# zhangyk18/GeoBi-GNN

Hardware: AMD Instinct MI355X
Metric: M-edges/s (fwd+bwd) on Synthetic set (higher is better)
Workload: dtype f32; 1 GPU; Synthetic train, batch=4 meshes (~20k faces each), fwd+bwd [BASELINE.json configs[2]]: per rank 4 noisy icospheres n=32 (F=20480) as one disjoint-union graph, L1/L1 loss, grad all-reduce + Adam step inside the timed region; ONE resident batch replayed every step, its level-0 CSR / reverse-edge index / corner lists / loss weights built in warm-up and cached per mesh (with --full, extra.fresh_batch:; meshes_per_rank=4, edges_per_rank_step=1351448, parallelism=dp1, mesh_groups_in_flight=1, split_allreduce=False, collective=none

## Files before the change

### geobi_gnn_amd/csrc/head_fused.hip

```cpp
#include "common.h"

#include <cstdlib>

namespace geobi {

namespace {

typedef float f32x16 __attribute__((ext_vector_type(16)));

constexpr int CIN = 32;
constexpr int HID = 1024;
constexpr int NCHUNK = HID / 32;
constexpr float kEps = 1e-12f;

__device__ __forceinline__ int acc_row(int r, int half) { return (r & 3) + 8 * (r >> 2) + 4 * half; }

__device__ __forceinline__ void load16(const float* __restrict__ p, float (&v)[16]) {
  const float4* q = reinterpret_cast<const float4*>(p);
#pragma unroll
  for (int i = 0; i < 4; ++i) {
    float4 t = q[i];
    v[4 * i] = t.x; v[4 * i + 1] = t.y; v[4 * i + 2] = t.z; v[4 * i + 3] = t.w;
  }
}

template <int NOUT>
__global__ __launch_bounds__(256) void head_fwd_fused_kernel(
    const float* __restrict__ x, int N, const float* __restrict__ w1, const float* __restrict__ b1,
    const float* __restrict__ w2, const float* __restrict__ b2, float slope, int mode,
    const float* __restrict__ dd, const float* __restrict__ resid, int ld_resid, float* __restrict__ raw,
    float* __restrict__ out) {
  __shared__ float s_part[4][32][NOUT + 1];
  const int lane = threadIdx.x & 63, wave = threadIdx.x >> 6;
  const int half = lane >> 5, l31 = lane & 31;
  const int n0 = blockIdx.x * 32;
  const int row = min(n0 + l31, N - 1);
  float ax[16];
  load16(x + (size_t)row * CIN + 16 * half, ax);

  float part[16][NOUT];
#pragma unroll
  for (int r = 0; r < 16; ++r)
#pragma unroll
    for (int o = 0; o < NOUT; ++o) part[r][o] = 0.f;

  auto chunk = [&](int c, const float (&bw)[16]) {
    const int j = c * 32 + l31;
    f32x16 acc;
#pragma unroll
    for (int r = 0; r < 16; ++r) acc[r] = 0.f;
#pragma unroll
    for (int s = 0; s < 16; ++s) acc = __builtin_amdgcn_mfma_f32_32x32x2f32(ax[s], bw[s], acc, 0, 0, 0);
    const float b1v = b1[j];
    float w2v[NOUT];
#pragma unroll
    for (int o = 0; o < NOUT; ++o) w2v[o] = w2[(size_t)o * HID + j];
#pragma unroll
    for (int r = 0; r < 16; ++r) {
      float h = acc[r] + b1v;
      h = h > 0.f ? h : h * slope;
#pragma unroll
      for (int o = 0; o < NOUT; ++o) part[r][o] = fmaf(h, w2v[o], part[r][o]);
    }
  };
  const float* w1l = w1 + (size_t)l31 * CIN + 16 * half;
  float bwa[16], bwb[16];
  load16(w1l + (size_t)wave * 32 * CIN, bwa);
  for (int c = wave; c < NCHUNK; c += 8) {
    load16(w1l + (size_t)(c + 4) * 32 * CIN, bwb);
    chunk(c, bwa);
    if (c + 8 < NCHUNK) load16(w1l + (size_t)(c + 8) * 32 * CIN, bwa);
    chunk(c + 4, bwb);
  }
#pragma unroll
  for (int r = 0; r < 16; ++r)
#pragma unroll
    for (int o = 0; o < NOUT; ++o) {
      float v = part[r][o];
#pragma unroll
      for (int m = 16; m >= 1; m >>= 1) v += __shfl_xor(v, m, 64);
      part[r][o] = v;
    }
#pragma unroll
  for (int r = 0; r < 16; ++r) {
    if (l31 != r) continue;
#pragma unroll
    for (int o = 0; o < NOUT; ++o) s_part[wave][acc_row(r, half)][o] = part[r][o];
  }
  __syncthreads();
  if (threadIdx.x < 32) {
    const int node = n0 + threadIdx.x;
    if (node >= N) return;
    float v[NOUT];
#pragma unroll
    for (int o = 0; o < NOUT; ++o) {
      v[o] = ((s_part[0][threadIdx.x][o] + s_part[1][threadIdx.x][o]) + s_part[2][threadIdx.x][o]) +
             s_part[3][threadIdx.x][o] + b2[o];
      raw[(size_t)node * NOUT + o] = v[o];
    }
    float res[3];
    if (mode == 0) {
#pragma unroll
      for (int cidx = 0; cidx < 3; ++cidx) {
        float t = (NOUT == 3) ? v[cidx % NOUT] : v[0] * dd[(size_t)node * 3 + cidx];
        res[cidx] = t + resid[(size_t)node * ld_resid + cidx];
      }
    } else {
      float len = fmaxf(sqrtf(v[0] * v[0] + v[1 % NOUT] * v[1 % NOUT] + v[2 % NOUT] * v[2 % NOUT]), kEps);
#pragma unroll
      for (int cidx = 0; cidx < 3; ++cidx) res[cidx] = v[cidx % NOUT] / len;
    }
    out[(size_t)node * 3] = res[0]; out[(size_t)node * 3 + 1] = res[1]; out[(size_t)node * 3 + 2] = res[2];
  }
}

typedef __bf16 bf16x8 __attribute__((ext_vector_type(8)));

struct Split3 { bf16x8 p[3]; };

__device__ __forceinline__ Split3 split3(const float (&v)[8]) {
  Split3 o;
#pragma unroll
  for (int j = 0; j < 8; ++j) {
    const __bf16 a = (__bf16)v[j];
    const float r1 = v[j] - (float)a;
    const __bf16 b = (__bf16)r1;
    const float r2 = r1 - (float)b;
    o.p[0][j] = a; o.p[1][j] = b; o.p[2][j] = (__bf16)r2;
  }
  return o;
}

__device__ __forceinline__ void load8(const float* __restrict__ p, float (&v)[8]) {
  const float4* q = reinterpret_cast<const float4*>(p);
  const float4 a = q[0], b = q[1];
  v[0] = a.x; v[1] = a.y; v[2] = a.z; v[3] = a.w; v[4] = b.x; v[5] = b.y; v[6] = b.z; v[7] = b.w;
}

__device__ __forceinline__ f32x16 mfma6(const Split3& a, const Split3& b, f32x16 acc) {
  acc = __builtin_amdgcn_mfma_f32_32x32x16_bf16(a.p[2], b.p[0], acc, 0, 0, 0);
  acc = __builtin_amdgcn_mfma_f32_32x32x16_bf16(a.p[0], b.p[2], acc, 0, 0, 0);
  acc = __builtin_amdgcn_mfma_f32_32x32x16_bf16(a.p[1], b.p[1], acc, 0, 0, 0);
  acc = __builtin_amdgcn_mfma_f32_32x32x16_bf16(a.p[1], b.p[0], acc, 0, 0, 0);
  acc = __builtin_amdgcn_mfma_f32_32x32x16_bf16(a.p[0], b.p[1], acc, 0, 0, 0);
  acc = __builtin_amdgcn_mfma_f32_32x32x16_bf16(a.p[0], b.p[0], acc, 0, 0, 0);
  return acc;
}

__global__ void head_split_w1_kernel(const float* __restrict__ w1, __bf16* __restrict__ pk) {
  const int i = blockIdx.x * blockDim.x + threadIdx.x;
  if (i >= HID * CIN) return;
  const float v = w1[i];
  const __bf16 a = (__bf16)v;
  const float r1 = v - (float)a;
  const __bf16 b = (__bf16)r1;
  pk[i] = a; pk[HID * CIN + i] = b; pk[2 * HID * CIN + i] = (__bf16)(r1 - (float)b);
}

__device__ __forceinline__ Split3 load_split(const __bf16* __restrict__ pk, size_t off) {
  Split3 o;
#pragma unroll
  for (int p = 0; p < 3; ++p) o.p[p] = *reinterpret_cast<const bf16x8*>(pk + (size_t)p * HID * CIN + off);
  return o;
}

template <int NOUT>
__global__ __launch_bounds__(256) void head_fwd_fused_bf16x3_kernel(
    const float* __restrict__ x, int N, const __bf16* __restrict__ w1p, const float* __restrict__ b1,
    const float* __restrict__ w2, const float* __restrict__ b2, float slope, int mode,
    const float* __restrict__ dd, const float* __restrict__ resid, int ld_resid, float* __restrict__ raw,
    float* __restrict__ out) {
  __shared__ float s_part[4][32][NOUT + 1];
  const int lane = threadIdx.x & 63, wave = threadIdx.x >> 6;
  const int half = lane >> 5, l31 = lane & 31;
  const int n0 = blockIdx.x * 32;
  const int row = min(n0 + l31, N - 1);
  Split3 ax[2];
  {
    float v[8];
    load8(x + (size_t)row * CIN + 8 * half, v);      ax[0] = split3(v);
    load8(x + (size_t)row * CIN + 16 + 8 * half, v); ax[1] = split3(v);
  }
  float part[16][NOUT];
#pragma unroll
  for (int r = 0; r < 16; ++r)
#pragma unroll
    for (int o = 0; o < NOUT; ++o) part[r][o] = 0.f;

  auto chunk = [&](int c, const Split3& bw0, const Split3& bw1) {
    const int j = c * 32 + l31;
    f32x16 acc;
#pragma unroll
    for (int r = 0; r < 16; ++r) acc[r] = 0.f;
    acc = mfma6(ax[0], bw0, acc);
    acc = mfma6(ax[1], bw1, acc);
    const float b1v = b1[j];
    float w2v[NOUT];
#pragma unroll
    for (int o = 0; o < NOUT; ++o) w2v[o] = w2[(size_t)o * HID + j];
#pragma unroll
    for (int r = 0; r < 16; ++r) {
      float h = acc[r] + b1v;
      h = h > 0.f ? h : h * slope;
#pragma unroll
      for (int o = 0; o < NOUT; ++o) part[r][o] = fmaf(h, w2v[o], part[r][o]);
    }
  };
  const size_t wl = (size_t)l31 * CIN + 8 * half;
  Split3 wa0 = load_split(w1p, wl + (size_t)wave * 32 * CIN), wa1 = load_split(w1p, wl + (size_t)wave * 32 * CIN + 16);
  for (int c = wave; c < NCHUNK; c += 8) {
    const Split3 wb0 = load_split(w1p, wl + (size_t)(c + 4) * 32 * CIN), wb1 = load_split(w1p, wl + (size_t)(c + 4) * 32 * CIN + 16);
    chunk(c, wa0, wa1);
    if (c + 8 < NCHUNK) { wa0 = load_split(w1p, wl + (size_t)(c + 8) * 32 * CIN); wa1 = load_split(w1p, wl + (size_t)(c + 8) * 32 * CIN + 16); }
    chunk(c + 4, wb0, wb1);
  }
#pragma unroll
  for (int r = 0; r < 16; ++r)
#pragma unroll
    for (int o = 0; o < NOUT; ++o) {
      float v = part[r][o];
#pragma unroll
      for (int m = 16; m >= 1; m >>= 1) v += __shfl_xor(v, m, 64);
      part[r][o] = v;
    }
#pragma unroll
  for (int r = 0; r < 16; ++r) {
    if (l31 != r) continue;
#pragma unroll
    for (int o = 0; o < NOUT; ++o) s_part[wave][acc_row(r, half)][o] = part[r][o];
  }
  __syncthreads();
  if (threadIdx.x < 32) {
    const int node = n0 + threadIdx.x;
    if (node >= N) return;
    float v[NOUT];
#pragma unroll
    for (int o = 0; o < NOUT; ++o) {
      v[o] = ((s_part[0][threadIdx.x][o] + s_part[1][threadIdx.x][o]) + s_part[2][threadIdx.x][o]) +
             s_part[3][threadIdx.x][o] + b2[o];
      raw[(size_t)node * NOUT + o] = v[o];
    }
    float res[3];
    if (mode == 0) {
#pragma unroll
      for (int cidx = 0; cidx < 3; ++cidx) {
        float t = (NOUT == 3) ? v[cidx % NOUT] : v[0] * dd[(size_t)node * 3 + cidx];
        res[cidx] = t + resid[(size_t)node * ld_resid + cidx];
      }
    } else {
      float len = fmaxf(sqrtf(v[0] * v[0] + v[1 % NOUT] * v[1 % NOUT] + v[2 % NOUT] * v[2 % NOUT]), kEps);
#pragma unroll
      for (int cidx = 0; cidx < 3; ++cidx) res[cidx] = v[cidx % NOUT] / len;
    }
    out[(size_t)node * 3] = res[0]; out[(size_t)node * 3 + 1] = res[1]; out[(size_t)node * 3 + 2] = res[2];
  }
}

#ifdef GEOBI_HEAD_STAMPS
__device__ unsigned long long g_head_stamps[1024][8];
#define GEOBI_HS(i) do { const unsigned long long now_ = __builtin_amdgcn_s_memtime(); hs_acc[i] += now_ - hs_t; hs_t = now_; } while (0)
#else
#define GEOBI_HS(i) do { } while (0)
#endif

constexpr int HBW = 8;
constexpr int HCPW = NCHUNK / HBW;

template <int NOUT>
__global__ __launch_bounds__(512, 1) void head_bwd_fused_kernel(
    const float* __restrict__ x, int N, int ntiles, const float* __restrict__ w1, const float* __restrict__ b1,
    const float* __restrict__ w2, float slope, const float* __restrict__ graw, float* __restrict__ dx,
    float* __restrict__ p_dw1, float* __restrict__ p_dw2, float* __restrict__ p_db1, float* __restrict__ p_db2) {
  extern __shared__ __attribute__((aligned(16))) float lds[];
  float* sW1 = lds;
  float* sW2 = sW1 + NCHUNK * 16 * 64;
  float* sB1 = sW2 + 3 * HID;
  float* sT = sB1 + HID;
  const int lane = threadIdx.x & 63, wave = threadIdx.x >> 6;
  const int half = lane >> 5, l31 = lane & 31;
  for (int i = threadIdx.x; i < NCHUNK * 16 * 64 + 3 * HID + HID; i += 64 * HBW) lds[i] = 0.f;
  __syncthreads();

  float db2a[NOUT];
#pragma unroll
  for (int o = 0; o < NOUT; ++o) db2a[o] = 0.f;
  float* tw = sT + wave * 512;
#ifdef GEOBI_HEAD_STAMPS
  unsigned long long hs_acc[8] = {0, 0, 0, 0, 0, 0, 0, 0};
  unsigned long long hs_t = __builtin_amdgcn_s_memtime();
#endif

  for (int t = blockIdx.x; t < ntiles; t += gridDim.x) {
    const int n0 = t * 32;
    float ax[16], ax2[16], gr[16][NOUT];
    load16(x + (size_t)min(n0 + l31, N - 1) * CIN + 16 * half, ax);
#pragma unroll
    for (int r = 0; r < 16; ++r) {
      const int node = n0 + acc_row(r, half);
      const bool ok = node < N;
      ax2[r] = x[(size_t)(ok ? node : N - 1) * CIN + l31];
#pragma unroll
      for (int o = 0; o < NOUT; ++o) {
        gr[r][o] = ok ? graw[(size_t)node * NOUT + o] : 0.f;
        db2a[o] += gr[r][o];
      }
    }
    f32x16 dxacc;
#pragma unroll
    for (int r = 0; r < 16; ++r) dxacc[r] = 0.f;
    GEOBI_HS(0);

    float bw[16];
    load16(w1 + (size_t)(wave * 32 + l31) * CIN + 16 * half, bw);
    for (int cc = 0; cc < HCPW; ++cc) {
      const int c = wave + HBW * cc;
      const int j = c * 32 + l31;
      f32x16 acc;
#pragma unroll
      for (int r = 0; r < 16; ++r) acc[r] = 0.f;
#pragma unroll
      for (int s = 0; s < 16; ++s) acc = __builtin_amdgcn_mfma_f32_32x32x2f32(ax[s], bw[s], acc, 0, 0, 0);
      GEOBI_HS(1);
      float bq[16];
      const float* wq = w1 + (size_t)(c * 32 + 16 * half) * CIN + l31;
#pragma unroll
      for (int s = 0; s < 16; ++s) bq[s] = wq[s * CIN];
      const float b1v = b1[j];
      float w2v[NOUT], dw2c[NOUT];
#pragma unroll
      for (int o = 0; o < NOUT; ++o) { w2v[o] = w2[(size_t)o * HID + j]; dw2c[o] = 0.f; }
      load16(w1 + (size_t)((wave + HBW * ((cc + 1) % HCPW)) * 32 + l31) * CIN + 16 * half, bw);
      float dh[16];
      float db1c = 0.f;
#pragma unroll
      for (int r = 0; r < 16; ++r) {
        float hpre = acc[r] + b1v;
        float hval = hpre > 0.f ? hpre : hpre * slope;
        float gh = 0.f;
#pragma unroll
        for (int o = 0; o < NOUT; ++o) {
          gh = fmaf(gr[r][o], w2v[o], gh);
          dw2c[o] = fmaf(gr[r][o], hval, dw2c[o]);
        }
        dh[r] = hpre > 0.f ? gh : gh * slope;
        db1c += dh[r];
      }
      GEOBI_HS(2);
      f32x16 tacc;
#pragma unroll
      for (int r = 0; r < 16; ++r) tacc[r] = 0.f;
#pragma unroll
      for (int r = 0; r < 16; ++r) tacc = __builtin_amdgcn_mfma_f32_32x32x2f32(ax2[r], dh[r], tacc, 0, 0, 0);
      float ad[16];
#pragma unroll
      for (int pass = 0; pass < 2; ++pass) {
#pragma unroll
        for (int r8 = 0; r8 < 8; ++r8) {
          const int r = 8 * pass + r8;
          const int row = acc_row(r, half) - 16 * pass;
          tw[row * 32 + (l31 ^ ((row & 7) << 2))] = dh[r];
        }
        __builtin_amdgcn_fence(__ATOMIC_RELEASE, "wavefront");
        __builtin_amdgcn_wave_barrier();
        __builtin_amdgcn_fence(__ATOMIC_ACQUIRE, "wavefront");
        if ((l31 >> 4) == pass) {
          const int row = l31 & 15;
#pragma unroll
          for (int q = 0; q < 4; ++q) {
            float4 v = *reinterpret_cast<const float4*>(&tw[row * 32 + ((16 * half + 4 * q) ^ ((row & 7) << 2))]);
            ad[4 * q] = v.x; ad[4 * q + 1] = v.y; ad[4 * q + 2] = v.z; ad[4 * q + 3] = v.w;
          }
        }
        __builtin_amdgcn_fence(__ATOMIC_RELEASE, "wavefront");
        __builtin_amdgcn_wave_barrier();
        __builtin_amdgcn_fence(__ATOMIC_ACQUIRE, "wavefront");
      }
      GEOBI_HS(3);
#pragma unroll
      for (int s = 0; s < 16; ++s) dxacc = __builtin_amdgcn_mfma_f32_32x32x2f32(ad[s], bq[s], dxacc, 0, 0, 0);
      GEOBI_HS(4);
      db1c += __shfl_xor(db1c, 32, 64);
      if (half == 0) sB1[j] += db1c;
#pragma unroll
      for (int o = 0; o < NOUT; ++o) {
        float d = dw2c[o] + __shfl_xor(dw2c[o], 32, 64);
        if (half == 0) sW2[o * HID + j] += d;
      }
      float* w1c = sW1 + (size_t)c * 16 * 64 + lane;
#pragma unroll
      for (int r = 0; r < 16; ++r) w1c[r * 64] += tacc[r];
      GEOBI_HS(5);
    }
#pragma unroll
    for (int hr = 0; hr < 2; ++hr) {
      __syncthreads();
#pragma unroll
      for (int r8 = 0; r8 < 8; ++r8) sT[(wave * 8 + r8) * 64 + lane] = dxacc[8 * hr + r8];
      __syncthreads();
      {
        const int r8 = wave;
        float v = 0.f;
#pragma unroll
        for (int w = 0; w < HBW; ++w) v += sT[(w * 8 + r8) * 64 + lane];
        const int node = n0 + acc_row(8 * hr + r8, half);
        if (node < N) dx[(size_t)node * CIN + l31] = v;
      }
    }
    __syncthreads();
    GEOBI_HS(6);
  }
#ifdef GEOBI_HEAD_STAMPS
  if (threadIdx.x == 0 && blockIdx.x < 1024)
    for (int i = 0; i < 8; ++i) g_head_stamps[blockIdx.x][i] = hs_acc[i];
#endif

  __syncthreads();
  float* pw = p_dw1 + (size_t)blockIdx.x * (NCHUNK * 16 * 64);
  for (int i = threadIdx.x; i < NCHUNK * 16 * 64; i += 64 * HBW) pw[i] = sW1[i];
  for (int i = threadIdx.x; i < NOUT * HID; i += 64 * HBW) p_dw2[(size_t)blockIdx.x * NOUT * HID + i] = sW2[i];
  for (int i = threadIdx.x; i < HID; i += 64 * HBW) p_db1[(size_t)blockIdx.x * HID + i] = sB1[i];
  if (wave == 0) {
#pragma unroll
    for (int o = 0; o < NOUT; ++o) {
      float d = db2a[o] + __shfl_xor(db2a[o], 32, 64);
      if (lane == 0) p_db2[(size_t)blockIdx.x * 4 + o] = d;
    }
  }
}

__global__ __launch_bounds__(256) void head_bwd_reduce_kernel(const float* __restrict__ p_dw1, const float* __restrict__ p_dw2,
                                       const float* __restrict__ p_db1, const float* __restrict__ p_db2,
                                       int blocks, int nout, int accumulate, float* __restrict__ dw1,
                                       float* __restrict__ db1, float* __restrict__ dw2, float* __restrict__ db2) {
  __shared__ float part[4][64];
  const int o = threadIdx.x & 63, q = threadIdx.x >> 6;
  const int idx = blockIdx.x * 64 + o;
  const int n_dw1 = HID * CIN;
  const int total = n_dw1 + HID + nout * HID + nout;
  const float* src = nullptr;
  size_t stride = 0, off = 0;
  float* dst = nullptr;
  if (idx < n_dw1) {
    const int c = idx >> 10, r = (idx >> 6) & 15, lane = idx & 63;
    const int j = c * 32 + (lane & 31), k = acc_row(r, lane >> 5);
    src = p_dw1; stride = (size_t)NCHUNK * 16 * 64; off = idx; dst = dw1 + (size_t)j * CIN + k;
  } else if (idx < n_dw1 + HID) {
    src = p_db1; stride = HID; off = idx - n_dw1; dst = db1 + off;
  } else if (idx < n_dw1 + HID + nout * HID) {
    src = p_dw2; stride = (size_t)nout * HID; off = idx - n_dw1 - HID; dst = dw2 + off;
  } else if (idx < total) {
    src = p_db2; stride = 4; off = idx - n_dw1 - HID - nout * HID; dst = db2 + off;
  }
  float s = 0.f;
  if (src != nullptr) {
#pragma unroll 16
    for (int b = q; b < blocks; b += 4) s += src[(size_t)b * stride + off];
  }
  part[q][o] = s;
  __syncthreads();
  if (q == 0 && dst != nullptr) {
    const float t = ((part[0][o] + part[1][o]) + part[2][o]) + part[3][o];
    *dst = accumulate ? *dst + t : t;
  }
}

int bwd_blocks(int64_t N) {
  int ntiles = cdiv(N, 32);
  return ntiles < 256 ? ntiles : 256;
}

}

#ifdef GEOBI_HEAD_STAMPS
extern "C" int geobi_debug_head_stamps(void* host_dst, size_t bytes) {
  return (int)hipMemcpyFromSymbol(host_dst, HIP_SYMBOL(g_head_stamps), bytes, 0, hipMemcpyDeviceToHost);
}
#endif

bool head_fused_supported(int Cin, int K, int nout) { return Cin == CIN && K == HID && (nout == 1 || nout == 3); }

static std::atomic<int> g_head_precision{[] { const char* e = getenv("GEOBI_HEAD_BF16X3"); return (e && atoi(e) != 0) ? 1 : 0; }()};
int set_head_precision(int mode) {
  GEOBI_REQUIRE(mode == 0 || mode == 1, "head precision: 0 (fp32) or 1 (3 x bf16 split, six products)");
  g_head_precision = mode;
  return 0;
}

int head_fwd_fused(const float* x, int64_t N, const float* w1, const float* b1, const float* w2, const float* b2,
                   int nout, float slope, int mode, const float* dd, const float* resid, int ld_resid, float* raw,
                   float* out, hipStream_t s) {
  int blocks = cdiv(N, 32);
  if (g_head_precision.load(std::memory_order_relaxed) == 1) {
    static thread_local __bf16* pack = nullptr;
    if (pack == nullptr) GEOBI_HIP(hipMalloc((void**)&pack, (size_t)3 * HID * CIN * sizeof(__bf16)));
    head_split_w1_kernel<<<cdiv(HID * CIN, 256), 256, 0, s>>>(w1, pack);
    if (nout == 3)
      head_fwd_fused_bf16x3_kernel<3><<<blocks, 256, 0, s>>>(x, (int)N, pack, b1, w2, b2, slope, mode, dd, resid, ld_resid,
                                                             raw, out);
    else
      head_fwd_fused_bf16x3_kernel<1><<<blocks, 256, 0, s>>>(x, (int)N, pack, b1, w2, b2, slope, mode, dd, resid, ld_resid,
                                                             raw, out);
    GEOBI_LAUNCH_OK();
    return 0;
  }
  if (nout == 3)
    head_fwd_fused_kernel<3><<<blocks, 256, 0, s>>>(x, (int)N, w1, b1, w2, b2, slope, mode, dd, resid, ld_resid, raw,
                                                    out);
  else
    head_fwd_fused_kernel<1><<<blocks, 256, 0, s>>>(x, (int)N, w1, b1, w2, b2, slope, mode, dd, resid, ld_resid, raw,
                                                    out);
  GEOBI_LAUNCH_OK();
  return 0;
}

size_t head_bwd_fused_ws_bytes(int64_t N) {
  size_t b = bwd_blocks(N);
  return align_up(b * (size_t)NCHUNK * 16 * 64 * sizeof(float)) + align_up(b * 3 * HID * sizeof(float)) +
         align_up(b * HID * sizeof(float)) + align_up(b * 4 * sizeof(float)) + 1024;
}

int head_bwd_fused(const float* x, int64_t N, const float* w1, const float* b1, const float* w2, int nout,
                   float slope, const float* graw, float* dx, float* dw1, float* db1, float* dw2, float* db2,
                   int accumulate, void* ws, size_t ws_bytes, hipStream_t s) {
  const int blocks = bwd_blocks(N);
  Arena a(ws, ws_bytes);
  float* p_dw1 = a.take<float>((size_t)blocks * NCHUNK * 16 * 64);
  float* p_dw2 = a.take<float>((size_t)blocks * 3 * HID);
  float* p_db1 = a.take<float>((size_t)blocks * HID);
  float* p_db2 = a.take<float>((size_t)blocks * 4);
  GEOBI_REQUIRE(a.ok() && ws, "head_bwd_fused: workspace too small (%zu < %zu)", ws_bytes, a.off);
  const int ntiles = cdiv(N, 32);
  constexpr size_t kLds = (size_t)(NCHUNK * 16 * 64 + 3 * HID + HID + HBW * 16 * 32) * sizeof(float);
  static_assert(kLds == 163840, "the backward head kernel uses the whole LDS of a CU");
  static std::atomic<bool> attr_set{false};
  if (!attr_set) {
    GEOBI_HIP(hipFuncSetAttribute((const void*)head_bwd_fused_kernel<3>, hipFuncAttributeMaxDynamicSharedMemorySize,
                                  (int)kLds));
    GEOBI_HIP(hipFuncSetAttribute((const void*)head_bwd_fused_kernel<1>, hipFuncAttributeMaxDynamicSharedMemorySize,
                                  (int)kLds));
    attr_set = true;
  }
  if (nout == 3)
    head_bwd_fused_kernel<3><<<blocks, 64 * HBW, kLds, s>>>(x, (int)N, ntiles, w1, b1, w2, slope, graw, dx, p_dw1, p_dw2,
                                                       p_db1, p_db2);
  else
    head_bwd_fused_kernel<1><<<blocks, 64 * HBW, kLds, s>>>(x, (int)N, ntiles, w1, b1, w2, slope, graw, dx, p_dw1, p_dw2,
                                                       p_db1, p_db2);
  GEOBI_LAUNCH_OK();
  const int total = HID * CIN + HID + nout * HID + nout;
  head_bwd_reduce_kernel<<<cdiv(total, 64), 256, 0, s>>>(p_dw1, p_dw2, p_db1, p_db2, blocks, nout, accumulate, dw1, db1,
                                                          dw2, db2);
  GEOBI_LAUNCH_OK();
  return 0;
}

}
```

Before: 328.8 M-edges/s.

## Add tiled head forward and multi-subtile backward kernels with register-resident dW2/dB1

New measurement: 333.3 M-edges/s, median of 4. +1.4%, better.

```diff
diff --git a/geobi_gnn_amd/csrc/head_fused.hip b/geobi_gnn_amd/csrc/head_fused.hip
--- a/geobi_gnn_amd/csrc/head_fused.hip
+++ b/geobi_gnn_amd/csrc/head_fused.hip
@@ -96,6 +96,141 @@
     for (int o = 0; o < NOUT; ++o) {
       v[o] = ((s_part[0][threadIdx.x][o] + s_part[1][threadIdx.x][o]) + s_part[2][threadIdx.x][o]) +
              s_part[3][threadIdx.x][o] + b2[o];
+      raw[(size_t)node * NOUT + o] = v[o];
+    }
+    float res[3];
+    if (mode == 0) {
+#pragma unroll
+      for (int cidx = 0; cidx < 3; ++cidx) {
+        float t = (NOUT == 3) ? v[cidx % NOUT] : v[0] * dd[(size_t)node * 3 + cidx];
+        res[cidx] = t + resid[(size_t)node * ld_resid + cidx];
+      }
+    } else {
+      float len = fmaxf(sqrtf(v[0] * v[0] + v[1 % NOUT] * v[1 % NOUT] + v[2 % NOUT] * v[2 % NOUT]), kEps);
+#pragma unroll
+      for (int cidx = 0; cidx < 3; ++cidx) res[cidx] = v[cidx % NOUT] / len;
+    }
+    out[(size_t)node * 3] = res[0]; out[(size_t)node * 3 + 1] = res[1]; out[(size_t)node * 3 + 2] = res[2];
+  }
+}
+
+constexpr int W1S = CIN + 4;
+
+template <int NOUT, int NT>
+__device__ __forceinline__ void fetch_chunk(const float* __restrict__ w1, const float* __restrict__ b1,
+                                            const float* __restrict__ w2, int c, int tid, float4 (&st)[256 / NT],
+                                            float (&sb)[((1 + NOUT) * 32 + NT - 1) / NT]) {
+  constexpr int NB = (1 + NOUT) * 32;
+  const float4* src = reinterpret_cast<const float4*>(w1 + (size_t)c * 32 * CIN);
+#pragma unroll
+  for (int i = 0; i < 256 / NT; ++i) st[i] = src[tid + i * NT];
+#pragma unroll
+  for (int i = 0; i < (NB + NT - 1) / NT; ++i) {
+    const int e = min(tid + i * NT, NB - 1), o = e >> 5, j = c * 32 + (e & 31);
+    sb[i] = o == 0 ? b1[j] : w2[(size_t)(o - 1) * HID + j];
+  }
+}
+
+template <int NOUT, int NT>
+__device__ __forceinline__ void stage_chunk(float* __restrict__ sw, float* __restrict__ sbw, int tid,
+                                            const float4 (&st)[256 / NT],
+                                            const float (&sb)[((1 + NOUT) * 32 + NT - 1) / NT]) {
+  constexpr int NB = (1 + NOUT) * 32;
+#pragma unroll
+  for (int i = 0; i < 256 / NT; ++i) {
+    const int idx = tid + i * NT;
+    *reinterpret_cast<float4*>(&sw[(idx >> 3) * W1S + 4 * (idx & 7)]) = st[i];
+  }
+#pragma unroll
+  for (int i = 0; i < (NB + NT - 1) / NT; ++i) {
+    const int e = tid + i * NT;
+    if (e < NB) sbw[e] = sb[i];
+  }
+}
+
+template <int NOUT, int NW>
+__global__ __launch_bounds__(64 * NW) void head_fwd_tile_kernel(
+    const float* __restrict__ x, int N, const float* __restrict__ w1, const float* __restrict__ b1,
+    const float* __restrict__ w2, const float* __restrict__ b2, float slope, int mode,
+    const float* __restrict__ dd, const float* __restrict__ resid, int ld_resid, float* __restrict__ raw,
+    float* __restrict__ out) {
+  constexpr int NT = 64 * NW;
+  constexpr int PER = 256 / NT;
+  constexpr int NB = (1 + NOUT) * 32;
+  constexpr int PERB = (NB + NT - 1) / NT;
+  __shared__ __attribute__((aligned(16))) float s_w1[2][32 * W1S];
+  __shared__ float s_bw[2][NB];
+  __shared__ float s_out[NW][32][NOUT + 1];
+  const int tid = threadIdx.x, lane = tid & 63, wave = tid >> 6;
+  const int half = lane >> 5, l31 = lane & 31;
+  const int n0 = (blockIdx.x * NW + wave) * 32;
+  const bool live = n0 < N;
+  float ax[16];
+  load16(x + (size_t)min(n0 + l31, N - 1) * CIN + 16 * half, ax);
+
+  float part[16][NOUT];
+#pragma unroll
+  for (int r = 0; r < 16; ++r)
+#pragma unroll
+    for (int o = 0; o < NOUT; ++o) part[r][o] = 0.f;
+
+  float4 st[PER];
+  float sb[PERB];
+  fetch_chunk<NOUT, NT>(w1, b1, w2, 0, tid, st, sb);
+  stage_chunk<NOUT, NT>(s_w1[0], s_bw[0], tid, st, sb);
+  __syncthreads();
+  for (int c = 0; c < NCHUNK; ++c) {
+    const int buf = c & 1;
+    fetch_chunk<NOUT, NT>(w1, b1, w2, min(c + 1, NCHUNK - 1), tid, st, sb);
+    if (live) {
+      float bw[16];
+      load16(&s_w1[buf][l31 * W1S + 16 * half], bw);
+      f32x16 acc;
+#pragma unroll
+      for (int r = 0; r < 16; ++r) acc[r] = 0.f;
+#pragma unroll
+      for (int s = 0; s < 16; ++s) acc = __builtin_amdgcn_mfma_f32_32x32x2f32(ax[s], bw[s], acc, 0, 0, 0);
+      const float b1v = s_bw[buf][l31];
+      float w2v[NOUT];
+#pragma unroll
+      for (int o = 0; o < NOUT; ++o) w2v[o] = s_bw[buf][32 * (o + 1) + l31];
+#pragma unroll
+      for (int r = 0; r < 16; ++r) {
+        float h = acc[r] + b1v;
+        h = h > 0.f ? h : h * slope;
+#pragma unroll
+        for (int o = 0; o < NOUT; ++o) part[r][o] = fmaf(h, w2v[o], part[r][o]);
+      }
+    }
+    stage_chunk<NOUT, NT>(s_w1[buf ^ 1], s_bw[buf ^ 1], tid, st, sb);
+    __syncthreads();
+  }
+  if (!live) return;
+#pragma unroll
+  for (int r = 0; r < 16; ++r)
+#pragma unroll
+    for (int o = 0; o < NOUT; ++o) {
+      float v = part[r][o];
+#pragma unroll
+      for (int m = 16; m >= 1; m >>= 1) v += __shfl_xor(v, m, 64);
+      part[r][o] = v;
+    }
+#pragma unroll
+  for (int r = 0; r < 16; ++r) {
+    if (l31 != r) continue;
+#pragma unroll
+    for (int o = 0; o < NOUT; ++o) s_out[wave][acc_row(r, half)][o] = part[r][o];
+  }
+  __builtin_amdgcn_fence(__ATOMIC_RELEASE, "wavefront");
+  __builtin_amdgcn_wave_barrier();
+  __builtin_amdgcn_fence(__ATOMIC_ACQUIRE, "wavefront");
+  if (lane < 32) {
+    const int node = n0 + lane;
+    if (node >= N) return;
+    float v[NOUT];
+#pragma unroll
+    for (int o = 0; o < NOUT; ++o) {
+      v[o] = s_out[wave][lane][o] + b2[o];
       raw[(size_t)node * NOUT + o] = v[o];
     }
     float res[3];
@@ -423,6 +558,216 @@
 #pragma unroll
     for (int o = 0; o < NOUT; ++o) {
       float d = db2a[o] + __shfl_xor(db2a[o], 32, 64);
+      if (lane == 0) p_db2[(size_t)blockIdx.x * 4 + o] = d;
+    }
+  }
+}
+
+constexpr int XS = CIN + 4;
+
+template <int NOUT, int NS>
+__global__ __launch_bounds__(512, 1) void head_bwd_tile_kernel(
+    const float* __restrict__ x, int N, int ntiles, const float* __restrict__ w1, const float* __restrict__ b1,
+    const float* __restrict__ w2, float slope, const float* __restrict__ graw, float* __restrict__ dx,
+    float* __restrict__ p_dw1, float* __restrict__ p_dw2, float* __restrict__ p_db1, float* __restrict__ p_db2) {
+  extern __shared__ __attribute__((aligned(16))) float lds[];
+  float* sW1 = lds;
+  float* sT = sW1 + NCHUNK * 16 * 64;
+  float* sX = sT + HBW * 16 * 32;
+  float* sG = sX + 32 * NS * XS;
+  const int lane = threadIdx.x & 63, wave = threadIdx.x >> 6;
+  const int half = lane >> 5, l31 = lane & 31;
+  for (int i = threadIdx.x; i < NCHUNK * 16 * 64; i += 64 * HBW) lds[i] = 0.f;
+
+  float db2a[NOUT], dw2a[HCPW][NOUT], db1a[HCPW];
+#pragma unroll
+  for (int o = 0; o < NOUT; ++o) db2a[o] = 0.f;
+#pragma unroll
+  for (int k = 0; k < HCPW; ++k) {
+    db1a[k] = 0.f;
+#pragma unroll
+    for (int o = 0; o < NOUT; ++o) dw2a[k][o] = 0.f;
+  }
+  float* tw = sT + wave * 512;
+  float* twr[4];
+#pragma unroll
+  for (int r3 = 0; r3 < 4; ++r3) twr[r3] = tw + (r3 + 4 * half) * 32 + (l31 ^ ((r3 + 4 * half) << 2));
+
+  float bw[16];
+  load16(w1 + (size_t)(wave * 32 + l31) * CIN + 16 * half, bw);
+
+  for (int t = blockIdx.x; t < ntiles; t += gridDim.x) {
+    const int n0 = t * 32 * NS;
+    __syncthreads();
+    for (int i = threadIdx.x; i < 32 * NS * 8; i += 64 * HBW) {
+      const int r = i >> 3, q = i & 7, node = n0 + r;
+      float4 v = make_float4(0.f, 0.f, 0.f, 0.f);
+      if (node < N) v = *reinterpret_cast<const float4*>(x + (size_t)node * CIN + 4 * q);
+      *reinterpret_cast<float4*>(&sX[r * XS + 4 * q]) = v;
+    }
+    for (int i = threadIdx.x; i < 32 * NS; i += 64 * HBW) {
+      const int node = n0 + i;
+      float g[4] = {0.f, 0.f, 0.f, 0.f};
+      if (node < N) {
+#pragma unroll
+        for (int o = 0; o < NOUT; ++o) g[o] = graw[(size_t)node * NOUT + o];
+      }
+#pragma unroll
+      for (int o = 0; o < NOUT; ++o) db2a[o] += g[o];
+      *reinterpret_cast<float4*>(&sG[i * 4]) = make_float4(g[0], g[1], g[2], g[3]);
+    }
+    __syncthreads();
+
+    f32x16 dxacc[NS];
+#pragma unroll
+    for (int s = 0; s < NS; ++s)
+#pragma unroll
+      for (int r = 0; r < 16; ++r) dxacc[s][r] = 0.f;
+
+#pragma unroll 1
+    for (int cc = 0; cc < HCPW; ++cc) {
+      const int c = wave + HBW * cc;
+      const int j = c * 32 + l31;
+      float bq[16];
+      const float* wq = w1 + (size_t)(c * 32 + 16 * half) * CIN + l31;
+#pragma unroll
+      for (int s = 0; s < 16; ++s) bq[s] = wq[s * CIN];
+      const float b1v = b1[j];
+      float w2v[NOUT], dw2c[NOUT];
+#pragma unroll
+      for (int o = 0; o < NOUT; ++o) { w2v[o] = w2[(size_t)o * HID + j]; dw2c[o] = 0.f; }
+      float db1c = 0.f;
+      f32x16 tacc;
+#pragma unroll
+      for (int r = 0; r < 16; ++r) tacc[r] = 0.f;
+
+#pragma unroll
+      for (int s = 0; s < NS; ++s) {
+        asm volatile("" ::: "memory");
+        __builtin_amdgcn_sched_barrier(0);
+        const float* xs = sX + 32 * s * XS;
+        const float* gs = sG + 32 * s * 4;
+        float ax[16];
+        load16(xs + l31 * XS + 16 * half, ax);
+        f32x16 acc;
+#pragma unroll
+        for (int r = 0; r < 16; ++r) acc[r] = 0.f;
+#pragma unroll
+        for (int k = 0; k < 16; ++k) acc = __builtin_amdgcn_mfma_f32_32x32x2f32(ax[k], bw[k], acc, 0, 0, 0);
+        if (s == NS - 1)
+          load16(w1 + (size_t)((wave + HBW * ((cc + 1) % HCPW)) * 32 + l31) * CIN + 16 * half, bw);
+        float dh[16];
+        float4 gn[2];
+#pragma unroll
+        for (int i = 0; i < 2; ++i) gn[i] = *reinterpret_cast<const float4*>(gs + acc_row(i, half) * 4);
+#pragma unroll
+        for (int rg = 0; rg < 8; ++rg) {
+          float4 gc[2];
+#pragma unroll
+          for (int i = 0; i < 2; ++i) gc[i] = gn[i];
+          if (rg < 7) {
+#pragma unroll
+            for (int i = 0; i < 2; ++i) gn[i] = *reinterpret_cast<const float4*>(gs + acc_row(2 * rg + 2 + i, half) * 4);
+          }
+          __builtin_amdgcn_sched_barrier(0);
+#pragma unroll
+          for (int i = 0; i < 2; ++i) {
+            const int r = 2 * rg + i;
+            const float gr[3] = {gc[i].x, gc[i].y, gc[i].z};
+            float hpre = acc[r] + b1v;
+            float hval = hpre > 0.f ? hpre : hpre * slope;
+            float gh = 0.f;
+#pragma unroll
+            for (int o = 0; o < NOUT; ++o) {
+              gh = fmaf(gr[o], w2v[o], gh);
+              dw2c[o] = fmaf(gr[o], hval, dw2c[o]);
+            }
+            dh[r] = hpre > 0.f ? gh : gh * slope;
+            db1c += dh[r];
+          }
+        }
+        __builtin_amdgcn_sched_barrier(0);
+        float ax2[16];
+#pragma unroll
+        for (int r = 0; r < 16; ++r) ax2[r] = xs[acc_row(r, half) * XS + l31];
+#pragma unroll
+        for (int r = 0; r < 16; ++r) tacc = __builtin_amdgcn_mfma_f32_32x32x2f32(ax2[r], dh[r], tacc, 0, 0, 0);
+        float ad[16];
+#pragma unroll
+        for (int pass = 0; pass < 2; ++pass) {
+#pragma unroll
+          for (int r8 = 0; r8 < 8; ++r8)
+            twr[r8 & 3][(r8 >> 2) * 256] = dh[8 * pass + r8];
+          __builtin_amdgcn_fence(__ATOMIC_RELEASE, "wavefront");
+          __builtin_amdgcn_wave_barrier();
+          __builtin_amdgcn_fence(__ATOMIC_ACQUIRE, "wavefront");
+          if ((l31 >> 4) == pass) {
+            const int row = l31 & 15;
+#pragma unroll
+            for (int q = 0; q < 4; ++q) {
+              float4 v = *reinterpret_cast<const float4*>(&tw[row * 32 + ((16 * half + 4 * q) ^ ((row & 7) << 2))]);
+              ad[4 * q] = v.x; ad[4 * q + 1] = v.y; ad[4 * q + 2] = v.z; ad[4 * q + 3] = v.w;
+            }
+          }
+          __builtin_amdgcn_fence(__ATOMIC_RELEASE, "wavefront");
+          __builtin_amdgcn_wave_barrier();
+          __builtin_amdgcn_fence(__ATOMIC_ACQUIRE, "wavefront");
+        }
+#pragma unroll
+        for (int k = 0; k < 16; ++k) dxacc[s] = __builtin_amdgcn_mfma_f32_32x32x2f32(ad[k], bq[k], dxacc[s], 0, 0, 0);
+      }
+      {
+        const float t0 = db1a[0] + db1c;
+        db1a[0] = db1a[1]; db1a[1] = db1a[2]; db1a[2] = db1a[3]; db1a[3] = t0;
+#pragma unroll
+        for (int o = 0; o < NOUT; ++o) {
+          const float t1 = dw2a[0][o] + dw2c[o];
+          dw2a[0][o] = dw2a[1][o]; dw2a[1][o] = dw2a[2][o]; dw2a[2][o] = dw2a[3][o]; dw2a[3][o] = t1;
+        }
+      }
+      float* w1c = sW1 + (size_t)c * 16 * 64 + lane;
+#pragma unroll
+      for (int r = 0; r < 16; ++r) w1c[r * 64] += tacc[r];
+    }
+#pragma unroll
+    for (int s = 0; s < NS; ++s)
+#pragma unroll
+      for (int hr = 0; hr < 2; ++hr) {
+        __syncthreads();
+#pragma unroll
+        for (int r8 = 0; r8 < 8; ++r8) sT[(wave * 8 + r8) * 64 + lane] = dxacc[s][8 * hr + r8];
+        __syncthreads();
+        {
+          const int r8 = wave;
+          float v = 0.f;
+#pragma unroll
+          for (int w = 0; w < HBW; ++w) v += sT[(w * 8 + r8) * 64 + lane];
+          const int node = n0 + 32 * s + acc_row(8 * hr + r8, half);
+          if (node < N) dx[(size_t)node * CIN + l31] = v;
+        }
+      }
+  }
+
+  __syncthreads();
+  float* pw = p_dw1 + (size_t)blockIdx.x * (NCHUNK * 16 * 64);
+  for (int i = threadIdx.x; i < NCHUNK * 16 * 64; i += 64 * HBW) pw[i] = sW1[i];
+#pragma unroll
+  for (int k = 0; k < HCPW; ++k) {
+    const int j = (wave + HBW * k) * 32 + l31;
+    const float d1 = db1a[k] + __shfl_xor(db1a[k], 32, 64);
+    if (half == 0) p_db1[(size_t)blockIdx.x * HID + j] = d1;
+#pragma unroll
+    for (int o = 0; o < NOUT; ++o) {
+      const float d = dw2a[k][o] + __shfl_xor(dw2a[k][o], 32, 64);
+      if (half == 0) p_dw2[(size_t)blockIdx.x * NOUT * HID + (size_t)o * HID + j] = d;
+    }
+  }
+  if (wave == 0) {
+#pragma unroll
+    for (int o = 0; o < NOUT; ++o) {
+      float d = db2a[o];
+#pragma unroll
+      for (int m = 32; m >= 1; m >>= 1) d += __shfl_xor(d, m, 64);
       if (lane == 0) p_db2[(size_t)blockIdx.x * 4 + o] = d;
     }
   }
@@ -464,10 +809,19 @@
   }
 }
 
-int bwd_blocks(int64_t N) {
-  int ntiles = cdiv(N, 32);
-  return ntiles < 256 ? ntiles : 256;
-}
+std::atomic<int> g_head_tiles{[] { const char* e = getenv("GEOBI_HEAD_TILES"); const int v = e ? atoi(e) : 1; return (v == 0 || v == 2) ? v : 1; }()};
+int head_tiles() { return g_head_tiles.load(std::memory_order_relaxed); }
+
+constexpr int kCUs = 256;
+
+int bwd_blocks(int64_t N, int ns = 1) {
+  int ntiles = cdiv(N, 32 * ns);
+  return ntiles < kCUs ? ntiles : kCUs;
+}
+
+int bwd_subtiles() { return head_tiles(); }
+
+int fwd_waves(int64_t N) { return N > 64 ? 4 : (N > 32 ? 2 : 1); }
 
 }
 
@@ -486,10 +840,25 @@
   return 0;
 }
 
+template <int NOUT, int NW, typename... A>
+static void launch_fwd_tile(int64_t N, hipStream_t s, A... a) {
+  head_fwd_tile_kernel<NOUT, NW><<<cdiv(N, 32 * NW), 64 * NW, 0, s>>>(a...);
+}
+
 int head_fwd_fused(const float* x, int64_t N, const float* w1, const float* b1, const float* w2, const float* b2,
                    int nout, float slope, int mode, const float* dd, const float* resid, int ld_resid, float* raw,
                    float* out, hipStream_t s) {
   int blocks = cdiv(N, 32);
+  if (head_tiles() == 2 && g_head_precision.load(std::memory_order_relaxed) == 0) {
+    const int nw = fwd_waves(N);
+#define GEOBI_FWD_TILE(NOUT_, NW_) \
+    launch_fwd_tile<NOUT_, NW_>(N, s, x, (int)N, w1, b1, w2, b2, slope, mode, dd, resid, ld_resid, raw, out)
+    if (nout == 3) { if (nw == 4) GEOBI_FWD_TILE(3, 4); else if (nw == 2) GEOBI_FWD_TILE(3, 2); else GEOBI_FWD_TILE(3, 1); }
+    else           { if (nw == 4) GEOBI_FWD_TILE(1, 4); else if (nw == 2) GEOBI_FWD_TILE(1, 2); else GEOBI_FWD_TILE(1, 1); }
+#undef GEOBI_FWD_TILE
+    GEOBI_LAUNCH_OK();
+    return 0;
+  }
   if (g_head_precision.load(std::memory_order_relaxed) == 1) {
     static thread_local __bf16* pack = nullptr;
     if (pack == nullptr) GEOBI_HIP(hipMalloc((void**)&pack, (size_t)3 * HID * CIN * sizeof(__bf16)));
@@ -514,7 +883,7 @@
 }
 
 size_t head_bwd_fused_ws_bytes(int64_t N) {
-  size_t b = bwd_blocks(N);
+  size_t b = bwd_blocks(N, bwd_subtiles() == 2 ? 2 : 1);
   return align_up(b * (size_t)NCHUNK * 16 * 64 * sizeof(float)) + align_up(b * 3 * HID * sizeof(float)) +
          align_up(b * HID * sizeof(float)) + align_up(b * 4 * sizeof(float)) + 1024;
 }
@@ -522,13 +891,42 @@
 int head_bwd_fused(const float* x, int64_t N, const float* w1, const float* b1, const float* w2, int nout,
                    float slope, const float* graw, float* dx, float* dw1, float* db1, float* dw2, float* db2,
                    int accumulate, void* ws, size_t ws_bytes, hipStream_t s) {
-  const int blocks = bwd_blocks(N);
+  const bool wide = bwd_subtiles() != 0;
+  const int ns = bwd_subtiles() == 2 ? 2 : 1;
+  const int blocks = bwd_blocks(N, ns);
   Arena a(ws, ws_bytes);
   float* p_dw1 = a.take<float>((size_t)blocks * NCHUNK * 16 * 64);
   float* p_dw2 = a.take<float>((size_t)blocks * 3 * HID);
   float* p_db1 = a.take<float>((size_t)blocks * HID);
   float* p_db2 = a.take<float>((size_t)blocks * 4);
   GEOBI_REQUIRE(a.ok() && ws, "head_bwd_fused: workspace too small (%zu < %zu)", ws_bytes, a.off);
+  const int total = HID * CIN + HID + nout * HID + nout;
+  if (wide) {
+    const int ntiles = cdiv(N, 32 * ns);
+    constexpr size_t kLdsBase = (size_t)(NCHUNK * 16 * 64 + HBW * 16 * 32) * sizeof(float);
+    const size_t lds_bytes = kLdsBase + (size_t)32 * ns * (XS + 4) * sizeof(float);
+    static_assert(kLdsBase + 64 * (XS + 4) * sizeof(float) <= 163840, "the wide backward tile must fit a CU's LDS");
+    static std::atomic<bool> tile_attr_set{false};
+    if (!tile_attr_set) {
+      const int cap = (int)(kLdsBase + 64 * (XS + 4) * sizeof(float));
+      GEOBI_HIP(hipFuncSetAttribute((const void*)head_bwd_tile_kernel<3, 2>, hipFuncAttributeMaxDynamicSharedMemorySize, cap));
+      GEOBI_HIP(hipFuncSetAttribute((const void*)head_bwd_tile_kernel<1, 2>, hipFuncAttributeMaxDynamicSharedMemorySize, cap));
+      GEOBI_HIP(hipFuncSetAttribute((const void*)head_bwd_tile_kernel<3, 1>, hipFuncAttributeMaxDynamicSharedMemorySize, cap));
+      GEOBI_HIP(hipFuncSetAttribute((const void*)head_bwd_tile_kernel<1, 1>, hipFuncAttributeMaxDynamicSharedMemorySize, cap));
+      tile_attr_set = true;
+    }
+#define GEOBI_BWD_TILE(NOUT_, NS_)                                                                                        \
+    head_bwd_tile_kernel<NOUT_, NS_><<<blocks, 64 * HBW, lds_bytes, s>>>(x, (int)N, ntiles, w1, b1, w2, slope, graw, dx, \
+                                                                         p_dw1, p_dw2, p_db1, p_db2)
+    if (nout == 3) { if (ns == 2) GEOBI_BWD_TILE(3, 2); else GEOBI_BWD_TILE(3, 1); }
+    else           { if (ns == 2) GEOBI_BWD_TILE(1, 2); else GEOBI_BWD_TILE(1, 1); }
+#undef GEOBI_BWD_TILE
+    GEOBI_LAUNCH_OK();
+    head_bwd_reduce_kernel<<<cdiv(total, 64), 256, 0, s>>>(p_dw1, p_dw2, p_db1, p_db2, blocks, nout, accumulate, dw1, db1,
+                                                            dw2, db2);
+    GEOBI_LAUNCH_OK();
+    return 0;
+  }
   const int ntiles = cdiv(N, 32);
   constexpr size_t kLds = (size_t)(NCHUNK * 16 * 64 + 3 * HID + HID + HBW * 16 * 32) * sizeof(float);
   static_assert(kLds == 163840, "the backward head kernel uses the whole LDS of a CU");
@@ -547,7 +945,6 @@
     head_bwd_fused_kernel<1><<<blocks, 64 * HBW, kLds, s>>>(x, (int)N, ntiles, w1, b1, w2, slope, graw, dx, p_dw1, p_dw2,
                                                        p_db1, p_db2);
   GEOBI_LAUNCH_OK();
-  const int total = HID * CIN + HID + nout * HID + nout;
   head_bwd_reduce_kernel<<<cdiv(total, 64), 256, 0, s>>>(p_dw1, p_dw2, p_db1, p_db2, blocks, nout, accumulate, dw1, db1,
                                                           dw2, db2);
   GEOBI_LAUNCH_OK();
@@ -555,3 +952,9 @@
 }
 
 }
+
+extern "C" int geobi_debug_head_tiles(int mode) {
+  const int prev = geobi::g_head_tiles.load();
+  if (mode >= 0 && mode <= 2) geobi::g_head_tiles = mode;
+  return prev;
+}
```
